# omangin/multimodal

Measured on AMD Instinct MI355X. Metric: nmf_update_iterations_per_sec, higher is better.
Workload: dtype f16 operands, fp32 accumulate; e4m3 ratio tiles and e4m3 W image in the H-numerator product

## Files before the change

### multimodal_amd/csrc/api_loop.hip

```cpp
#include "ctx.hip.h"

namespace klnmf_host {
namespace {

RowPass4Key rowpass4_key(const klnmf_ctx *c, int mode, bool tiles, int grid_y) {
    const bool upd = mode == ROW_UPDATE;
    const bool q8 = upd && c->q8() && tiles;
    const bool ne = q8 && c->ne_loop && !c->big;
    return RowPass4Key{c->KT, 2 * c->KT - c->ks, mode, c->kc >= 0 ? 1 : 0, c->big ? 4 : kWaves4, (upd && grid_y > 1) ? 1 : 0,
                       q8 ? (ne ? 2 : 1) : 0};
}

void launch_rowpass4_kt(klnmf_ctx *c, int mode, const RowPass4Args &a, int grid_x, int grid_y = 1) {
    struct Table {
        void (*slot[kRowPass4Count])(RowPass4Args) = {};
        Table() { KL_RP4_LIST_1(KL_RP4_SLOT) KL_RP4_LIST_2(KL_RP4_SLOT) KL_RP4_LIST_3(KL_RP4_SLOT) }
    };
    static const Table table;
    const RowPass4Key key = rowpass4_key(c, mode, a.base.Qt != nullptr, grid_y);
    if (mode == ROW_UPDATE) c->last_row_ne = key.q8 == 2;
    const int idx = rowpass4_index(key);
    if (idx < 0) fail(KLNMF_ERR_UNSUPP, "ping-pong row pass: 224 < k <= 256 runs on the generation-1 kernel");
    if (!table.slot[idx]) fail(KLNMF_ERR_UNSUPP, "ping-pong row pass: no kernel in slot " + std::to_string(idx));
    hipLaunchKernelGGL(table.slot[idx], dim3(grid_x, grid_y), dim3(64 * key.nw), 0, c->stream, a);
// ... 332 lines not shown
                           NumArray<T, 2>{{(const T *)c->Npart, (const T *)c->Dpart}}, OutSets<T, 2>{{(T *)c->numer, (T *)c->denom}},
                           count, c->nsplit, (const DevState *)c->st);
    else
        hipLaunchKernelGGL((k_sum_partials<T, 1>), dim3(grid_for(count)), dim3(256), 0, c->stream,
                           NumArray<T, 1>{{(const T *)c->Npart}}, OutSets<T, 1>{{(T *)c->numer}}, count, c->nsplit, (const DevState *)c->st);
    HIPCHK(hipGetLastError());
}

template <typename T>
void exact_H(klnmf_ctx *c, bool from_slabs = false) {
    auto rule = [&](auto fac) {
        typedef decltype(fac) Fac;
        typedef NumArray<T, Fac::S> Arr;
        typedef NumSlabs<T, Fac::S> Slabs;
        Arr sums{}, slab0{};
        const T *const psums[2] = {(const T *)c->numer, (const T *)c->denom}, *const pslabs[2] = {(const T *)c->Npart, (const T *)c->Dpart};
        for (int s = 0; s < Fac::S; ++s) { sums.p[s] = psums[s]; slab0.p[s] = pslabs[s]; }
        if (from_slabs) {
            hipLaunchKernelGGL((k_update_H<T, Slabs, Fac>), dim3((unsigned)c->k), dim3(256), 0, c->stream, (T *)c->H,
                               RuleIn<Slabs, Fac>{Slabs{slab0, c->nsplit, c->k * c->f}, fac}, c->f, (const DevState *)c->st);
        } else if (c->hseg_n > 1) {
            hipLaunchKernelGGL((k_update_H_part<T, Fac>), dim3((unsigned)c->hseg_n, (unsigned)c->k), dim3(256), 0, c->stream, (T *)c->H,
                               RuleIn<Arr, Fac>{sums, fac}, c->f, c->hseg, c->hpart, (const DevState *)c->st);
            hipLaunchKernelGGL((k_update_H_norm<T>), dim3((unsigned)c->hseg_n, (unsigned)c->k), dim3(256), 0, c->stream, (T *)c->H,
                               c->f, c->hseg, (const double *)c->hpart, (const DevState *)c->st);
        } else {
            hipLaunchKernelGGL((k_update_H<T, Arr, Fac>), dim3((unsigned)c->k), dim3(256), 0, c->stream, (T *)c->H, RuleIn<Arr, Fac>{sums, fac},
                               c->f, (const DevState *)c->st);
        }
        HIPCHK(hipGetLastError());
    };
    if (c->weighted()) rule(FacDen{});
    else if (c->presence()) rule(FacPresH<T>{(const T *)c->pres_D, (const unsigned char *)c->pres_mod, c->pres_M});
    else rule(FacNum{});
}

#define EXACT_CALL(c, fn, ...)                                         \
    do {                                                               \
        if ((c)->prec == KLNMF_PREC_F64) fn<double>(c, ##__VA_ARGS__); \
        else fn<float>(c, ##__VA_ARGS__);                              \
    } while (0)

}

void launch_monitor(klnmf_ctx *c, bool use8) {
    c->mon_pending = false;
    c->mon_dry_pending = false;
    if (!c->mon_part || !c->sw.q8_monitor || !c->q8_loop) return;
    const bool dry = c->iter_in_loop == 1 && !c->q8();
    if (!dry && !(c->q8() && monitor_due(c->stat_q8_tiles))) return;
    MonArgs a{};
    a.st = c->st; a.Qt = c->Qt; a.VtA = (const _Float16 *)c->VtA; a.W32_old = c->W32[c->cur]; a.H_old = c->H32;
    a.Wb_new = c->Wb[c->cur ^ 1]; a.W8 = (use8 && !dry) ? c->W8 : nullptr; a.w8s = c->w8s; a.part = c->mon_part;
    a.spread = c->mon_spread;
    a.dry = dry ? 1 : 0;
    a.w8tab = (dry && c->W8 != nullptr && c->conv_ran) ? c->w8tab : nullptr;
    a.nrt = c->nrt; a.nct = c->nct; a.kp = c->KP; a.k = (int)c->k; a.wld = (int)w_ld(c->KP); a.w8ld = (int)w8_ld(c->KP);
    a.f_pad = c->f_pad;
    const int tiles = (int)((c->f + 31) / 32);
    a.ct = (int)((c->mon_checks * 5 + 1) % tiles);
    a.ncols = (int)std::min<int64_t>(32, c->f - (int64_t)a.ct * 32);
    a.nrt_data = (int)((c->n + 31) / 32);
    a.nsamp = std::min(2 * kMonBlocks, a.nrt_data) & ~1;
    if (a.nsamp < 2) return;
    a.rot = (int)((c->mon_checks * 7) % a.nrt_data);
    a.eps = (float)(kEpsRatio * c->v_scale);
    hipLaunchKernelGGL(k_q8_monitor, dim3(2 * kMonBlocks), dim3(256), 0, c->stream, a);
    HIPCHK(hipGetLastError());
    c->mon_pending = true;
    c->mon_dry_pending = dry;
    c->mon_ncols = a.ncols;
    c->mon_noise_scale = (float)std::min(0.5, (double)(a.nsamp / 2) * 32.0 / (double)c->n);
    c->mon_checks += 1;
}

bool fused_w8_stage(klnmf_ctx *c) {
    c->conv_ran = false;
    if (!c->W8 || !c->q8_loop) return false;
    const bool measure_only = c->iter_in_loop == 1 && !c->w8_meas;
    if (!measure_only && !c->q8()) return false;
    const bool use8 = !measure_only && c->w8_meas;
    const int groups = c->KP / 8, rpb = std::max(1, 256 / groups);
    const int64_t rows = c->n_pad;
    const int blocks = (int)std::min<int64_t>((rows + rpb - 1) / rpb, kW8Blocks);
    hipLaunchKernelGGL(k_w8_from_wb, dim3(blocks), dim3(256), 0, c->stream, (const opnd_t *)c->Wb[c->cur ^ 1], c->W8, rows,
                       c->KP, (int)w_ld(c->KP), (const float *)c->w8s, (const DevState *)c->st,
                       &c->st->w8_sat, w8_probe_col(c), c->w8tab,
                       ((unsigned)c->sr_launches++ * 0x9E3779B9u + 0x7F4A7C15u) ^ ((unsigned)c->comm_rank * 0xC2B2AE35u));
    HIPCHK(hipGetLastError());
    c->w8_meas = true;
    c->conv_ran = true;
    return use8;
}

void fused_colpass_part(klnmf_ctx *c, const klnmf_ctx::PartCfg &p, bool use8) {
    ColPassQArgs a = colq_part_args(c, p);
    const int grid = p.ncb * p.nchunks;
    EventPair ev{};
    if (c->prof_now) ev = begin_event(c, c->ev_col);
    auto launch_q2 = [&](const ColPassQArgs &g, bool fp8_tiles) {
        switch (c->KT) {
#define KL_PQ2(KTV) case KTV:                                                                                                    \
            if (fp8_tiles) hipLaunchKernelGGL((k_colpass_q2<KTV, KL_COLQ8_NB, 1, 1, KL_COLQ8_PAIR>), dim3(grid), dim3(kThreads), 0, c->stream, g); \
            else hipLaunchKernelGGL((k_colpass_q2<KTV, KL_COLQ_NB>), dim3(grid), dim3(kThreads), 0, c->stream, g);                \
            break;
#define KL_PQ2_BIG(KTV) case KTV:                                                                                                \
            if (fp8_tiles) hipLaunchKernelGGL((k_colpass_q2<KTV, 3, 2, 1, 1>), dim3(grid), dim3(kThreads), 0, c->stream, g);      \
            else hipLaunchKernelGGL((k_colpass_q2<KTV, 3, 2>), dim3(grid), dim3(kThreads), 0, c->stream, g);                      \
            break;
            KL_PQ2(1) KL_PQ2(2) KL_PQ2(3) KL_PQ2(4) KL_PQ2(5) KL_PQ2(6) KL_PQ2(7)
            KL_PQ2_BIG(8) KL_PQ2_BIG(10) KL_PQ2_BIG(12) KL_PQ2_BIG(14) KL_PQ2_BIG(16)
#undef KL_PQ2
#undef KL_PQ2_BIG
            default: fail(KLNMF_ERR_UNSUPP, "stored-ratio column pass: k <= 224 or 256 < k <= 512");
        }
        HIPCHK(hipGetLastError());
    };
    if (use8) {
        a.guard = 1;
        ColPass8Args a8{a, c->W8, c->w8s, w8_probe_col(c) >= 0 ? 1 : 0};
        if (c->KT == 8 && !c->big) fail(KLNMF_ERR_UNSUPP, "fp8 x fp8 column pass: KT = 8 only on the component-split path");
        switch (c->KT) {
#define KL_PQ8X(KTV, NBV, KSV) case KTV:                                                                                          \
            if (a8.probe) hipLaunchKernelGGL((k_colpass_q8x<KTV, NBV, KSV, 1>), dim3(grid), dim3(kThreads), 0, c->stream, a8);     \
            else hipLaunchKernelGGL((k_colpass_q8x<KTV, NBV, KSV, 0>), dim3(grid), dim3(kThreads), 0, c->stream, a8);              \
            break;
            KL_PQ8X(1, KL_COL8_NB, 1) KL_PQ8X(2, KL_COL8_NB, 1) KL_PQ8X(3, KL_COL8_NB, 1) KL_PQ8X(4, KL_COL8_NB, 1)
            KL_PQ8X(5, KL_COL8_NB, 1) KL_PQ8X(6, KL_COL8_NB, 1) KL_PQ8X(7, KL_COL8_NB, 1)
            KL_PQ8X(8, 3, 2) KL_PQ8X(10, 3, 2) KL_PQ8X(12, 3, 2) KL_PQ8X(14, 3, 2) KL_PQ8X(16, 3, 2)
#undef KL_PQ8X
            default: fail(KLNMF_ERR_UNSUPP, "fp8 x fp8 column pass: k <= 224 or 256 < k <= 512");
        }
        HIPCHK(hipGetLastError());
        ColPassQArgs g = a;
        g.guard = 2;
        launch_q2(g, true);
    } else {
        launch_q2(a, c->q8());
    }
    if (c->prof_now) HIPCHK(hipEventRecord(ev.b, c->stream));
}

void launch_post(klnmf_ctx *c, PostMode mode, const klnmf_ctx::PartCfg *parts, int nparts, const LossArgs &la, bool decide,
                 bool use8, bool last_sum) {
    PostArgs a{};
    a.nparts = nparts;
    for (int p = 0; p < nparts; ++p) {
        const klnmf_ctx::PartCfg &q = parts[p];
        a.part[p] = PostPart{c->NpartF + q.slab_off, c->numerF + q.numer_off, (int64_t)c->KP * q.ld, q.ld, q.col0, q.ncols,
                             q.nchunks, q.ct0};
    }
    a.do_sum = mode != POST_RULE;
    a.do_rule = mode != POST_SUM;
    a.do_decide = decide ? 1 : 0;
    a.loss_from_parts = (mode == POST_FULL && la.part != nullptr) ? 1 : 0;
    a.loss_block = (mode == POST_SUM && la.part != nullptr) ? 1 : 0;
    a.w8_block = (a.do_sum && last_sum && c->conv_ran && c->w8tab != nullptr) ? 1 : 0;
    a.last_sum = (a.do_sum && last_sum) ? 1 : 0;
    a.it = (int)(c->iter_in_loop & 1);
    a.mon = MonPost{nullptr, nullptr, kMonMinSpread, kMonMaxCommon, 0, 0.f, kMonThreshold};
    if (a.do_sum && c->mon_pending) {
        a.mon = MonPost{c->mon_part, c->mon_spread, c->sw.mon_min_spread >= 0.f ? c->sw.mon_min_spread : kMonMinSpread,
                        c->sw.mon_threshold > 0.f ? 1.0f : kMonMaxCommon, c->mon_ncols,
                        c->mon_noise_scale, c->sw.mon_threshold > 0.f ? c->sw.mon_threshold : kMonThreshold};
        c->mon_pending = false;
    }
    const int nloss = (a.do_sum && la.part != nullptr)
                          ? (int)std::min<int64_t>(kLossRedMax, std::max<int64_t>(1, (la.count + kLossRedSlice - 1) / kLossRedSlice)) : 0;
    a.loss_red = c->loss_red; a.nloss = nloss; a.inv_c = la.inv_c; a.loss_xchg = c->loss_xchg; a.ne = la.ne; a.cq_on = la.cq_on;
    a.tol_abs = la.tol_abs; a.errors = c->errors; a.cap = c->cap;
    a.st = c->st;
    a.H_old = c->H32; a.H_new = c->H32alt;
    a.Ht4 = c->Ht4; a.hsum = c->hsum; a.tcur = c->tcur; a.t_hs = c->t_hs;
    a.f = c->f; a.f_pad = c->f_pad; a.kp = c->KP; a.k = (int)c->k; a.kc = c->kc;
    a.eps_pad = (float)(kEpsRatio * c->v_scale);
    const bool fix = a.do_sum && c->q8() && c->q8_list != nullptr && c->sw.q8_fixup;
    a.list = fix ? c->q8_list : nullptr;
    a.Qt = c->Qt; a.VtA = (const _Float16 *)c->VtA; a.W32_old = c->W32[c->cur]; a.Wb_new = c->Wb[c->cur ^ 1];
    a.W8 = use8 ? c->W8 : nullptr; a.w8s = c->w8s; a.w8ld = (int)w8_ld(c->KP); a.wld = (int)w_ld(c->KP);
    a.nrt = c->nrt; a.nct = c->nct; a.stages_per_chunk = nparts == 1 ? parts[0].spc : 0; a.eps = (float)(kEpsRatio * c->v_scale);
    a.w8tab = c->w8tab; a.w8s_next = c->w8s_next;
    if (a.do_sum && !fix && c->q8() && c->q8_list != nullptr)
        HIPCHK(hipMemsetAsync(&c->st->q8_list_n, 0, sizeof(int), c->stream));
    if (a.do_sum) {
        SlabSumArgs sa{};
        for (int p = 0; p < nparts; ++p) sa.part[p] = a.part[p];
        sa.nparts = nparts; sa.k = (int)c->k; sa.f_pad = c->f_pad; sa.nloss = nloss;
        sa.loss_part = la.part; sa.loss_count = la.count; sa.loss_red = c->loss_red; sa.st = c->st;
        hipLaunchKernelGGL(k_slab_sum, dim3((unsigned)((c->f_pad + 1023) / 1024), (unsigned)(c->k + nloss)), dim3(256), 0, c->stream, sa);
        HIPCHK(hipGetLastError());
    }
    const int hthreads = c->f_pad >= 4096 ? 1024 : (c->f_pad >= 2048 ? 512 : 256);
    const int blocks = (int)c->k + a.w8_block + a.loss_block;
    hipLaunchKernelGGL(k_post, dim3((unsigned)blocks), dim3(hthreads), 0, c->stream, a);
    HIPCHK(hipGetLastError());
    if (a.do_rule) {
        std::swap(c->H32, c->H32alt);
        c->loop_hswaps += 1;
        c->images_measured = false;
    }
    if (a.w8_block) {
        std::swap(c->w8s, c->w8s_next);
        c->conv_ran = false;
    }
}

bool fp8_poll_due(const klnmf_ctx *c) {
    if (c->is_exact() || !c->q8_loop) return false;
    if (c->mon_dry_pending) return true;
    const bool q8_then = c->iter_in_loop + 1 >= 2 && (!c->big || (c->W8 != nullptr && c->w8_meas));
    return q8_then && monitor_due(c->stat_q8_tiles);
}

// ... 489 lines not shown
```

### multimodal_amd/csrc/colq8x.hip.h

```cpp
#pragma once
#include "colq.hip.h"

#define KL_COL8_PF 1
#define KL_COL8_NB 4

namespace klnmf {

__host__ __device__ constexpr int w8_ld(int kp) { return kp + ((kp / 32) % 2 == 0 ? 32 : 0); }

KL_GLOBAL __launch_bounds__(256) void k_w8_from_wb(const opnd_t *Wb, unsigned char *W8, int64_t rows, int kp, int wld,
                                                    const float *w8s, const DevState *st, int *sat, int probe_col,
                                                    unsigned *tab64, unsigned sr_seed) {
    const int ld8 = w8_ld(kp);
    typedef __attribute__((ext_vector_type(2))) _Float16 f16x2;
    if (st->stop) return;
    KL_FP16_SATURATE();
    __shared__ float red[8][256 / 8 * 8];
    const int groups = kp / 8;
    const int c8 = threadIdx.x % groups, rl = threadIdx.x / groups;
    const int rows_per_block = blockDim.x / groups;
    const int comp = 8 * c8;
    f16x2 inv[4];
    float mx[8];
    int nsat = 0;
#pragma unroll
    for (int u = 0; u < 4; ++u) inv[u] = f16x2{(_Float16)(1.f / w8s[comp + 2 * u]), (_Float16)(1.f / w8s[comp + 2 * u + 1])};
#pragma unroll
    for (int e = 0; e < 8; ++e) mx[e] = 0.f;
    if (rl < rows_per_block) {
        const int64_t stride = (int64_t)gridDim.x * rows_per_block;
        constexpr int U = 4;
        for (int64_t row0 = (int64_t)blockIdx.x * rows_per_block + rl; row0 < rows; row0 += U * stride) {
            opx8 v[U];
#pragma unroll
            for (int q = 0; q < U; ++q) {
                const int64_t row = row0 + q * stride;
                if (row < rows) v[q] = *(const opx8 *)(Wb + row * wld + wb_col((int)(row & 31), comp));
            }
#pragma unroll
            for (int q = 0; q < U; ++q) {
                const int64_t row = row0 + q * stride;
                if (row >= rows) break;
                unsigned out[2];
#pragma unroll
                for (int u = 0; u < 2; ++u) {
                    const f16x2 p0 = f16x2{v[q][4 * u], v[q][4 * u + 1]} * inv[2 * u], p1 = f16x2{v[q][4 * u + 2], v[q][4 * u + 3]} * inv[2 * u + 1];
                    unsigned sd = ((unsigned)row * 0x9E3779B1u) ^ ((unsigned)(comp + 4 * u) * 0x85EBCA6Bu) ^ sr_seed;
                    sd = (sd ^ (sd >> 15)) * 0x2C1B3C6Du;
                    const unsigned r1 = (sd ^ (sd >> 12)) * 0x297A2D39u, r2 = (r1 & 0xffffffu) * 0x6C8E95u + 0x3C6EF35Fu;
                    int w = 0;
                    w = __builtin_amdgcn_cvt_scalef32_sr_fp8_f16(w, p0[0], r1, 1.f, 0);
                    w = __builtin_amdgcn_cvt_scalef32_sr_fp8_f16(w, p0[1], r1 << 7, 1.f, 1);
                    w = __builtin_amdgcn_cvt_scalef32_sr_fp8_f16(w, p1[0], r2, 1.f, 2);
                    w = __builtin_amdgcn_cvt_scalef32_sr_fp8_f16(w, p1[1], r2 << 7, 1.f, 3);
                    const f16x2 top = __builtin_elementwise_max(p0, p1);
                    nsat += (top[0] > (_Float16)448.f || top[1] > (_Float16)448.f) ? ((p0[0] > (_Float16)448.f) + (p0[1] > (_Float16)448.f)
                                                                                     + (p1[0] > (_Float16)448.f) + (p1[1] > (_Float16)448.f)) : 0;
                    out[u] = __builtin_bit_cast(unsigned, w);
                }
                if (probe_col >= comp && probe_col < comp + 8) {
                    const int pc = probe_col - comp;
                    out[pc >> 2] = (out[pc >> 2] & ~(0xffu << (8 * (pc & 3)))) | (0x38u << (8 * (pc & 3)));
                }
                *(uint2 *)(W8 + row * ld8 + comp) = make_uint2(out[0], out[1]);
#pragma unroll
                for (int e = 0; e < 8; ++e) mx[e] = fmaxf(mx[e], (float)v[q][e]);
            }
        }
    }
    if (sat != nullptr && nsat != 0) atomicAdd(sat, nsat);
#pragma unroll
    for (int e = 0; e < 8; ++e) red[e][threadIdx.x] = mx[e];
    __syncthreads();
    if (rl == 0) {
#pragma unroll
        for (int e = 0; e < 8; ++e) {
            float m = red[e][c8];
            for (int q = 1; q < rows_per_block; ++q) m = fmaxf(m, red[e][q * groups + c8]);
            atomicMax(tab64 + (int64_t)(blockIdx.x & 63) * kp + comp + e, __float_as_uint(m));
        }
    }
}

typedef __attribute__((ext_vector_type(2))) int i32x2_t;
template <int OFF>
__device__ __forceinline__ void lds_read_tr8(i32x2_t &dst, unsigned addr) {
    asm volatile("ds_read_b64_tr_b8 %0, %1 offset:%2" : "=v"(dst) : "v"(addr), "n"(OFF));
}

struct ColPass8Args {
    ColPassQArgs q;
    const unsigned char *W8;
    const float *w8s;
    int probe;
};



__device__ __forceinline__ float e4m3_value(unsigned b) {
    const int ex = (int)((b >> 3) & 15u), man = (int)(b & 7u);
    return ex == 0 ? ldexpf((float)man, -9) : ldexpf(1.f + 0.125f * (float)man, ex - 7);
}
template <int KT, int NB, int KSPLIT = 1, int PROBE = 1>
__global__ __launch_bounds__(kThreads, 1) void k_colpass_q8x(ColPass8Args aa) {
    const ColPassQArgs &a = aa.q;
    typedef __attribute__((ext_vector_type(8))) int i32x8;
    typedef i32x2_t i32x2;
    static_assert((KSPLIT == 1 || KSPLIT == 2) && KT % KSPLIT == 0, "wave decomposition");
    constexpr int CTW = kWavesPerWG / KSPLIT;
    constexpr int KTW = KT / KSPLIT;
    constexpr int KP = 32 * KT;
    constexpr int LD8 = w8_ld(KP);
    constexpr int WST = 64 * LD8;
    constexpr int WA = round_up(WST, kGldsRound);
    constexpr int WR = WA / kGldsRound;
    constexpr int QA = CTW * 2 * kQTile8;
    constexpr int OBJ = WA + QA;
    constexpr int QPW = 2 / KSPLIT;
    constexpr int OPS = WR + QPW;
    static_assert(NB >= 3 && NB <= 5 && NB * OBJ <= 160 * 1024, "LDS budget");
    __shared__ __attribute__((aligned(16))) unsigned char o0[OBJ];
    __shared__ __attribute__((aligned(16))) unsigned char o1[OBJ];
    __shared__ __attribute__((aligned(16))) unsigned char o2[OBJ];
    __shared__ __attribute__((aligned(16))) unsigned char o3[NB > 3 ? OBJ : 16];
    __shared__ __attribute__((aligned(16))) unsigned char o4[NB > 4 ? OBJ : 16];
    if (a.st->stop) return;
    if (a.guard == 1 && a.st->w8_sat != 0) return;

    const int tid = threadIdx.x, lane = tid & 63, wave = __builtin_amdgcn_readfirstlane(tid >> 6);
    const int r = lane & 31, h = lane >> 5;
    const int G = gridDim.x;
    int lin = blockIdx.x;
    if ((G & 7) == 0) lin = (blockIdx.x & 7) * (G >> 3) + (blockIdx.x >> 3);
    const int chunk = lin / a.ncb, cb = lin % a.ncb;
    const int ctl = wave % CTW, kh = wave / CTW;
    const int ct_raw = cb * CTW + ctl;
    const bool active = ct_raw < a.nct;
    const int ct = active ? ct_raw : a.nct - 1;
    const int sbeg = chunk * a.stages_per_chunk;
    const int send = min(a.nrt / 2, sbeg + a.stages_per_chunk);
    if (sbeg >= send) {
        if (active) {
            float *np = a.Npart + (int64_t)chunk * KP * a.f_pad + (int64_t)ct * 32 + r;
            for (int c = 32 * KTW * kh + h; c < 32 * KTW * (kh + 1); c += 2) np[(int64_t)c * a.f_pad] = 0.f;
        }
        return;
    }
    const int i16 = lane & 15, half = (lane >> 4) & 1;
    const unsigned off_a = (32 * h + (i16 >> 1)) * LD8 + 16 * half + 8 * (i16 & 1) + 32 * KTW * kh;
    const unsigned off_b = WA + (2 * ctl + h) * kQTile8 + (i16 >> 1) * 32 + 16 * half + 8 * (i16 & 1);

    f32x16 acc[KTW];
#pragma unroll
// ... 25 lines not shown
    float probe_prev = 0.f, probe_max = 0.f;
    unsigned q8_flag = 0u;

    auto compute = [&](unsigned base, int stage_row0) {
        (void)stage_row0;
        i32x2 bq[4];
        static_for<0, 4>([&](auto U) {
            constexpr int u = decltype(U)::value;
            lds_read_tr8<u * 8 * 32>(bq[u], base + off_b);
        });
        constexpr int PF = KL_COL8_PF < KTW ? KL_COL8_PF : (KTW > 1 ? KTW - 1 : 1);
        constexpr int RG = PF + 1;
        i32x2 ring[RG][4];
        auto fetch = [&](auto M) {
            constexpr int m = decltype(M)::value;
            if constexpr (m < KTW) {
                static_for<0, 4>([&](auto U) {
                    constexpr int u = decltype(U)::value;
                    lds_read_tr8<u * 8 * LD8 + 32 * (KTW - 1 - m)>(ring[m % RG][u], base + off_a);
                });
            }
        };
        static_for<0, PF>([&](auto M) { fetch(M); });
        constexpr int young0 = 4 * (PF < KTW ? PF : KTW);
        asm volatile("s_waitcnt lgkmcnt(%4)" : "+v"(bq[0]), "+v"(bq[1]), "+v"(bq[2]), "+v"(bq[3]) : "n"(young0));
        const i32x8 bo = {bq[0][0], bq[0][1], bq[1][0], bq[1][1], bq[2][0], bq[2][1], bq[3][0], bq[3][1]};
        static_for<0, KTW>([&](auto M) {
            constexpr int m = decltype(M)::value;
            fetch(std::integral_constant<int, m + PF>{});
            constexpr int young = 4 * ((m + PF < KTW ? m + PF : KTW - 1) - m);
            asm volatile("s_waitcnt lgkmcnt(%4)" : "+v"(ring[m % RG][0]), "+v"(ring[m % RG][1]), "+v"(ring[m % RG][2]), "+v"(ring[m % RG][3]) : "n"(young));
            const i32x8 ao = {ring[m % RG][0][0], ring[m % RG][0][1], ring[m % RG][1][0], ring[m % RG][1][1],
                              ring[m % RG][2][0], ring[m % RG][2][1], ring[m % RG][3][0], ring[m % RG][3][1]};
            acc[KTW - 1 - m] = __builtin_amdgcn_mfma_scale_f32_32x32x64_f8f6f4(ao, bo, acc[KTW - 1 - m], 0, 0, 0, 127, 0, 127);
            __builtin_amdgcn_sched_barrier(0);
        });
        {
            if constexpr (PROBE != 0) {
                const float now = acc[KTW - 1][15];
                probe_max = fmaxf(probe_max, now - probe_prev);
                probe_prev = now;
            } else {
#pragma unroll
                for (int e = 0; e < 8; ++e) q8_flag |= q8_sat_mask((unsigned)bo[e]);
            }
        }
    };
    auto fence = [&]() {
        __builtin_amdgcn_sched_barrier(0);
        asm volatile("s_waitcnt vmcnt(%0)\n\ts_barrier" ::"n"((NB - 2) * OPS) : "memory");
        __builtin_amdgcn_sched_barrier(0);
    };
    static_for<0, NB - 1>([&](auto I) { stage_in(decltype(I)::value, sbeg + decltype(I)::value); });
    fence();
    for (int s0 = sbeg; s0 < send; s0 += NB) {
        static_for<0, NB>([&](auto I) {
            constexpr int i = decltype(I)::value;
            if (s0 + i < send) {
                stage_in((i + NB - 1) % NB, s0 + i + NB - 1);
                compute(lds_addr(obj(i)), 64 * (s0 + i));
                fence();
            }
        });
    }
    asm volatile("s_waitcnt vmcnt(0)" ::: "memory");
    if (!active) return;
    if (a.q8_list != nullptr && kh == KSPLIT - 1) {
        bool mine;
        if (PROBE != 0) mine = h == 1 && probe_max >= 31.5f;
        else mine = h == 0 && (q8_flag | (unsigned)__shfl_xor((int)q8_flag, 32, 64)) != 0u;
        if (mine) q8_suspect_append(a.st_rw, a.q8_list, chunk, ct, r);
    }
    const int rcol = 8 * ((r >> 2) & 3) + 4 * (r >> 4) + (r & 3);
    float *np = a.Npart + (int64_t)chunk * KP * a.f_pad + (int64_t)ct * 32 + rcol;
#pragma unroll
    for (int m = 0; m < KTW; ++m)
#pragma unroll
        for (int e = 0; e < 16; ++e) {
            const int comp = 32 * (KTW * kh + m) + 8 * (e >> 2) + 4 * h + (e & 3);
            np[(int64_t)comp * a.f_pad] = acc[m][e] * (kQ8Scale * aa.w8s[comp]);
        }
}

}
```

### multimodal_amd/csrc/ctx.hip.h

```cpp
#pragma once
#include <hip/hip_runtime.h>
#include <dlfcn.h>
#include <rccl/rccl.h>

#include <algorithm>
#include <cmath>
#include <cstdio>
#include <cstdlib>
#include <cstring>
#include <functional>
#include <limits>
#include <map>
#include <mutex>
#include <stdexcept>
#include <string>
#include <type_traits>
#include <vector>

#include "../../include/klnmf.h"
#include "stage_chunks.h"
#include "common.hip.h"
#include "exact.hip.h"
#include "weighted.hip.h"
#include "presence.hip.h"
// ... 125 lines not shown
        if (it == free_blocks.end() || it->second.empty()) return nullptr;
        void *p = it->second.back();
        it->second.pop_back();
        held -= cls;
        return p;
    }
    void flush(int device) {
        std::lock_guard<std::mutex> g(mu);
        for (auto &kv : free_blocks) {
            if (kv.first.first != device) continue;
            for (void *p : kv.second) { (void)hipFree(p); held -= kv.first.second; }
            kv.second.clear();
        }
    }
    bool give(int device, size_t cls, void *p) {
        if (cls > ((size_t)64 << 20)) return false;
        std::lock_guard<std::mutex> g(mu);
        if (held + cls > limit()) return false;
        free_blocks[{device, cls}].push_back(p);
        held += cls;
        return true;
    }
};
extern DevBlockCache g_block_cache;

struct DeviceBlocks {
    int device = 0;
    hipStream_t stream = nullptr;
    std::vector<std::pair<void *, size_t>> allocs;
    void *dalloc(size_t bytes, bool zero = true) {
        if (bytes == 0) bytes = 16;
        const size_t cls = DevBlockCache::size_class(bytes);
        void *p = g_block_cache.take(device, cls);
        if (!p) {
            hipError_t e = hipMalloc(&p, cls);
            if (e == hipErrorOutOfMemory) {
                (void)hipGetLastError();
                g_block_cache.flush(device);
                e = hipMalloc(&p, cls);
            }
            HIPCHK(e);
        }
        allocs.push_back({p, cls});
        if (zero) HIPCHK(hipMemsetAsync(p, 0, bytes, stream));
        return p;
    }
    void dfree(void *&p) {
        for (size_t i = 0; i < allocs.size(); ++i) {
            if (allocs[i].first != p) continue;
            if (!g_block_cache.give(device, allocs[i].second, p)) (void)hipFree(p);
            allocs.erase(allocs.begin() + (std::ptrdiff_t)i);
            break;
        }
        p = nullptr;
    }
    void release_all() {
        for (auto &b : allocs)
            if (!g_block_cache.give(device, b.second, b.first)) (void)hipFree(b.first);
        allocs.clear();
    }
};

template <typename Place>
void staged_upload(hipStream_t stream, const void *src, size_t es, int64_t rows, int64_t cols, int64_t ld, Place &&place) {
    const int64_t rows_per = stage_rows_per(rows, ld, es);
    void *d = nullptr;
    HIPCHK(hipMalloc(&d, stage_alloc_bytes(rows_per, ld, es)));
    try {
        stage_walk(rows, cols, ld, es, rows_per, [&](const StageChunk &ch) {
            HIPCHK(hipMemcpyAsync(d, (const char *)src + ch.offset, ch.bytes, hipMemcpyHostToDevice, stream));
            place((const void *)d, ch.r0, ch.rr);
            HIPCHK(hipStreamSynchronize(stream));
        });
    } catch (...) {
        (void)hipFree(d);
        throw;
    }
    (void)hipFree(d);
}

struct DevSwitches {
    int qtile = 0;
    int col8 = -1;
    int ne = -1;
    bool q8_fixup = true;
    bool q8_monitor = true;
    float mon_threshold = 0.f, mon_min_spread = -1.f;
    bool ratio_scale = true;
    bool eps_pad = true;
    int row_split = -1;
    int row_tail = -1;
    int comm_parts = 1;
    bool comm_overlap = true;
    bool comm_single = false;
    int sp_cb = 0, sp_rb = 0;
    int ex_rc = 0, ex_wc = 0;
    int64_t ex_hseg = 0;
    static DevSwitches read() {
        DevSwitches d;
        auto num = [](const char *name, int dflt) { const char *e = std::getenv(name); return e ? std::atoi(e) : dflt; };
        if (num("KLNMF_QTILE", 0) == 16) d.qtile = 16;
        if (num("KLNMF_DEV", 0) == 0) return d;
        d.qtile = num("KLNMF_QTILE", 0);
        d.col8 = num("KLNMF_COL8", -1);
        d.ne = num("KLNMF_NE", -1);
        d.q8_fixup = num("KLNMF_Q8_FIXUP", 1) != 0;
        d.q8_monitor = num("KLNMF_Q8_MONITOR", 1) != 0;
        if (const char *e = std::getenv("KLNMF_MON_THRESHOLD")) d.mon_threshold = (float)std::atof(e);
        if (const char *e = std::getenv("KLNMF_MON_MIN_SPREAD")) d.mon_min_spread = (float)std::atof(e);
        d.ratio_scale = num("KLNMF_RATIO_SCALE", 1) != 0;
        d.eps_pad = num("KLNMF_NO_EPS_PAD", 0) == 0;
        d.row_split = num("KLNMF_ROW_SPLIT", -1);
        d.row_tail = num("KLNMF_ROW_TAIL", -1);
        d.comm_parts = num("KLNMF_COMM_PARTS", 1);
        d.comm_overlap = num("KLNMF_COMM_OVERLAP", 1) != 0;
        d.comm_single = num("KLNMF_COMM_SINGLE", 0) != 0;
        d.sp_cb = num("KLNMF_SP_CB", 0);
        d.sp_rb = num("KLNMF_SP_RB", 0);
        d.ex_rc = std::max(0, num("KLNMF_EX_ROW_CHUNKS", 0));
        d.ex_wc = std::max(0, num("KLNMF_EX_W_CHUNKS", 0));
        d.ex_hseg = std::max(0, num("KLNMF_EX_H_SEG", 0));
        return d;
    }
};

#include "plan.hip.h"

namespace klnmf_host {

struct ContextState : DeviceBlocks {
    int prec = KLNMF_PREC_F64;
    bool own_stream = false;
    int cu_count = 256;
    double ratio_eps = kEpsRatio;
    void *poll_host = nullptr;
    hipEvent_t poll_ev = nullptr;

    bool profiling = false;
    int profile_every = 1;
    int64_t profile_seq = 0;
    std::vector<EventPair> ev_row, ev_col, ev_tail;

    ncclComm_t comm = nullptr;
    int comm_rank = 0, comm_size = 1;
    double *comm_scratch = nullptr;
    hipStream_t comm_stream = nullptr;
    hipEvent_t ev_part[kPostMaxParts] = {}, ev_ar[kPostMaxParts] = {};
};

struct PresenceState {
    int pres_M = 0, pres_dchunks = 0;
    int64_t pres_bounds[kMaxMod + 1] = {};
    void *Pm = nullptr, *pres_S = nullptr, *pres_D = nullptr;
    void *pres_dbounds = nullptr, *pres_mod = nullptr, *pres_Dslab = nullptr;
    bool presence() const { return pres_M > 0; }
    void forget_presence() { *this = PresenceState(); }
};

struct ProblemState : ProblemPlan, PresenceState {
    DevSwitches sw;
    int64_t cap = 0;
    bool have_problem = false;
    int cur = 0;
    int loop_start_cur = 0;
    int64_t loop_hswaps = 0;
    float *loop_h0 = nullptr, *loop_h1 = nullptr;

    DevState *st = nullptr;
    double *errors = nullptr;
    double *loss_xchg = nullptr;
    double2 *loss_red = nullptr;

    void *V = nullptr, *W[2] = {nullptr, nullptr}, *H = nullptr, *Q = nullptr;
    void *Npart = nullptr, *numer = nullptr;
    double *loss_part = nullptr;
    void *Wpart = nullptr;
    void *Om = nullptr, *Dpart = nullptr, *denom = nullptr, *WDpart = nullptr;
    float *x3_hs = nullptr, *x3_qr = nullptr;
    unsigned *x3_xmax = nullptr;
    double *x3_loss = nullptr;

    int64_t *sp_indptr = nullptr, *sp_indices = nullptr, *csc_indptr = nullptr, *csc_rows = nullptr, *csc_perm = nullptr;
    void *sp_data = nullptr, *sp_q = nullptr, *HT = nullptr;
    double *sp_row_loss = nullptr, *sp_wpart = nullptr, *sp_prod = nullptr;
    int *sp_idx32 = nullptr, *csc_rows32 = nullptr, *csc_perm32 = nullptr;
    int64_t *sp_blkptr = nullptr, *csc_blkptr = nullptr;
    double *sp_loss_part = nullptr;
// ... 185 lines not shown
```

Baseline: 215.9.

## Software-pipeline W8 conversion kernel and add opt-in paired fp8 column pass

Rewrites the W-to-fp8 conversion kernel to double-buffer row loads across trips. It uses scalar base offsets and incrementally computed stochastic-rounding seeds, hoists the probe-column mask, and defers saturation counting behind a wave ballot. The per-row max is now tracked on raw f16 bits. A new column-pass kernel variant gives each wave two column tiles sharing one W operand fetch, but it runs only under a dev env switch. The pipelining adds register pressure and relies on static assumptions about row spacing.

```diff
diff --git a/multimodal_amd/csrc/api_loop.hip b/multimodal_amd/csrc/api_loop.hip
--- a/multimodal_amd/csrc/api_loop.hip
+++ b/multimodal_amd/csrc/api_loop.hip
@@ -438,6 +438,7 @@
     const bool use8 = !measure_only && c->w8_meas;
     const int groups = c->KP / 8, rpb = std::max(1, 256 / groups);
     const int64_t rows = c->n_pad;
+    static_assert(kW8Blocks % 16 == 0, "k_w8_from_wb: a thread's rows lie a multiple of 16 apart");
     const int blocks = (int)std::min<int64_t>((rows + rpb - 1) / rpb, kW8Blocks);
     hipLaunchKernelGGL(k_w8_from_wb, dim3(blocks), dim3(256), 0, c->stream, (const opnd_t *)c->Wb[c->cur ^ 1], c->W8, rows,
                        c->KP, (int)w_ld(c->KP), (const float *)c->w8s, (const DevState *)c->st,
@@ -481,10 +482,19 @@
             if (a8.probe) hipLaunchKernelGGL((k_colpass_q8x<KTV, NBV, KSV, 1>), dim3(grid), dim3(kThreads), 0, c->stream, a8);     \
             else hipLaunchKernelGGL((k_colpass_q8x<KTV, NBV, KSV, 0>), dim3(grid), dim3(kThreads), 0, c->stream, a8);              \
             break;
-            KL_PQ8X(1, KL_COL8_NB, 1) KL_PQ8X(2, KL_COL8_NB, 1) KL_PQ8X(3, KL_COL8_NB, 1) KL_PQ8X(4, KL_COL8_NB, 1)
-            KL_PQ8X(5, KL_COL8_NB, 1) KL_PQ8X(6, KL_COL8_NB, 1) KL_PQ8X(7, KL_COL8_NB, 1)
+#define KL_PQ8X1(KTV) case KTV:                                                                                                    \
+            if (c->sw.col8_pair == 1) {                                                                                            \
+                if (a8.probe) hipLaunchKernelGGL((k_colpass_q8x_pair<KTV, KL_COL8_NB, 1>), dim3(grid), dim3(kThreads), 0, c->stream, a8); \
+                else hipLaunchKernelGGL((k_colpass_q8x_pair<KTV, KL_COL8_NB, 0>), dim3(grid), dim3(kThreads), 0, c->stream, a8);   \
+                break;                                                                                                             \
+            }                                                                                                                      \
+            if (a8.probe) hipLaunchKernelGGL((k_colpass_q8x<KTV, KL_COL8_NB, 1, 1>), dim3(grid), dim3(kThreads), 0, c->stream, a8); \
+            else hipLaunchKernelGGL((k_colpass_q8x<KTV, KL_COL8_NB, 1, 0>), dim3(grid), dim3(kThreads), 0, c->stream, a8);         \
+            break;
+            KL_PQ8X(1, KL_COL8_NB, 1) KL_PQ8X1(2) KL_PQ8X1(3) KL_PQ8X1(4) KL_PQ8X1(5) KL_PQ8X1(6) KL_PQ8X1(7)
             KL_PQ8X(8, 3, 2) KL_PQ8X(10, 3, 2) KL_PQ8X(12, 3, 2) KL_PQ8X(14, 3, 2) KL_PQ8X(16, 3, 2)
 #undef KL_PQ8X
+#undef KL_PQ8X1
             default: fail(KLNMF_ERR_UNSUPP, "fp8 x fp8 column pass: k <= 224 or 256 < k <= 512");
         }
         HIPCHK(hipGetLastError());
diff --git a/multimodal_amd/csrc/colq8x.hip.h b/multimodal_amd/csrc/colq8x.hip.h
--- a/multimodal_amd/csrc/colq8x.hip.h
+++ b/multimodal_amd/csrc/colq8x.hip.h
@@ -1,5 +1,6 @@
 #pragma once
 #include "colq.hip.h"
+#include "w8_seed.h"
 
 #define KL_COL8_PF 1
 #define KL_COL8_NB 4
@@ -7,12 +8,52 @@
 namespace klnmf {
 
 __host__ __device__ constexpr int w8_ld(int kp) { return kp + ((kp / 32) % 2 == 0 ? 32 : 0); }
+
+typedef __attribute__((ext_vector_type(2))) _Float16 f16x2;
+typedef __attribute__((ext_vector_type(2))) short s16x2;
+__device__ __forceinline__ s16x2 w8_raw_pair(const opx8 &v, int u) {
+    return __builtin_bit_cast(s16x2, f16x2{v[2 * u], v[2 * u + 1]});
+}
+__device__ __forceinline__ int64_t w8_uniform(int64_t x) {
+    asm("" : "+s"(x));
+    return x;
+}
+struct W8Lane {
+    f16x2 inv[4];
+    unsigned keep[2], put[2];
+};
+__device__ __forceinline__ uint2 w8_convert_row(const opx8 &v, const W8Lane &ln, unsigned sd0, unsigned sd1, f16x2 &top) {
+    unsigned out[2];
+#pragma unroll
+    for (int u = 0; u < 2; ++u) {
+        const f16x2 p0 = f16x2{v[4 * u], v[4 * u + 1]} * ln.inv[2 * u], p1 = f16x2{v[4 * u + 2], v[4 * u + 3]} * ln.inv[2 * u + 1];
+        unsigned r1, r2;
+        w8_seed_mix(u == 0 ? sd0 : sd1, r1, r2);
+        asm("" : "+v"(r1));
+        int w = 0;
+        w = __builtin_amdgcn_cvt_scalef32_sr_fp8_f16(w, p0[0], r1, 1.f, 0);
+        w = __builtin_amdgcn_cvt_scalef32_sr_fp8_f16(w, p0[1], r1 << 7, 1.f, 1);
+        w = __builtin_amdgcn_cvt_scalef32_sr_fp8_f16(w, p1[0], r2, 1.f, 2);
+        w = __builtin_amdgcn_cvt_scalef32_sr_fp8_f16(w, p1[1], r2 << 7, 1.f, 3);
+        top = __builtin_elementwise_max(top, __builtin_elementwise_max(p0, p1));
+        out[u] = (__builtin_bit_cast(unsigned, w) & ln.keep[u]) | ln.put[u];
+    }
+    return make_uint2(out[0], out[1]);
+}
+__device__ __forceinline__ int w8_count_sat(const opx8 &v, const W8Lane &ln) {
+    int n = 0;
+#pragma unroll
+    for (int u = 0; u < 4; ++u) {
+        const f16x2 p = f16x2{v[2 * u], v[2 * u + 1]} * ln.inv[u];
+        n += (p[0] > (_Float16)448.f) + (p[1] > (_Float16)448.f);
+    }
+    return n;
+}
 
 KL_GLOBAL __launch_bounds__(256) void k_w8_from_wb(const opnd_t *Wb, unsigned char *W8, int64_t rows, int kp, int wld,
                                                     const float *w8s, const DevState *st, int *sat, int probe_col,
                                                     unsigned *tab64, unsigned sr_seed) {
     const int ld8 = w8_ld(kp);
-    typedef __attribute__((ext_vector_type(2))) _Float16 f16x2;
     if (st->stop) return;
     KL_FP16_SATURATE();
     __shared__ float red[8][256 / 8 * 8];
@@ -20,55 +61,81 @@
     const int c8 = threadIdx.x % groups, rl = threadIdx.x / groups;
     const int rows_per_block = blockDim.x / groups;
     const int comp = 8 * c8;
-    f16x2 inv[4];
+    W8Lane ln;
+    s16x2 mxp[4];
+    int nsat = 0;
+#pragma unroll
+    for (int u = 0; u < 4; ++u) {
+        ln.inv[u] = f16x2{(_Float16)(1.f / w8s[comp + 2 * u]), (_Float16)(1.f / w8s[comp + 2 * u + 1])};
+        mxp[u] = s16x2{0, 0};
+    }
+#pragma unroll
+    for (int u = 0; u < 2; ++u) {
+        const int pc = probe_col - (comp + 4 * u);
+        const bool here = pc >= 0 && pc < 4;
+        ln.keep[u] = here ? ~(0xffu << (8 * pc)) : ~0u;
+        ln.put[u] = here ? 0x38u << (8 * pc) : 0u;
+    }
+    if (rl < rows_per_block) {
+        constexpr int U = kW8RowsPerTrip;
+        const int64_t stride = (int64_t)gridDim.x * rows_per_block;
+        int64_t brow = (int64_t)blockIdx.x * rows_per_block;
+        const unsigned src_off = 2u * (unsigned)(rl * wld + wb_col((int)((brow + rl) & 31), comp));
+        const unsigned dst_off = (unsigned)(rl * ld8 + comp);
+        const int64_t src_row = 2 * (int64_t)wld, src_q = stride * src_row, dst_q = stride * ld8;
+        const char *const src = (const char *)Wb;
+        int64_t src_o = brow * src_row, dst_o = brow * ld8;
+        W8Seed seed(brow + rl, stride, comp, sr_seed);
+        auto load_trip = [&](opx8(&v)[U], int ahead) {
+#pragma unroll
+            for (int q = 0; q < U; ++q) v[q] = *(const opx8 *)(src + w8_uniform(src_o + (ahead * U + q) * src_q) + src_off);
+        };
+        auto convert_trip = [&](const opx8(&v)[U]) {
+            f16x2 top = f16x2{(_Float16)0.f, (_Float16)0.f};
+#pragma unroll
+            for (int q = 0; q < U; ++q) {
+                *(uint2 *)(W8 + w8_uniform(dst_o + q * dst_q) + dst_off) = w8_convert_row(v[q], ln, seed.at(q, 0), seed.at(q, 1), top);
+#pragma unroll
+                for (int u = 0; u < 4; ++u) mxp[u] = __builtin_elementwise_max(mxp[u], w8_raw_pair(v[q], u));
+            }
+            if (__builtin_amdgcn_ballot_w64(top[0] > (_Float16)448.f || top[1] > (_Float16)448.f) != 0) {
+#pragma unroll
+                for (int q = 0; q < U; ++q) nsat += w8_count_sat(v[q], ln);
+            }
+            brow += U * stride, src_o += U * src_q, dst_o += U * dst_q, seed.next_trip();
+        };
+        if (w8_full_trip(brow, stride, rows_per_block, rows)) {
+            opx8 va[U], vb[U];
+            load_trip(va, 0);
+            for (;;) {
+                if (!w8_full_trip(brow + U * stride, stride, rows_per_block, rows)) { convert_trip(va); break; }
+                load_trip(vb, 1);
+                convert_trip(va);
+                if (!w8_full_trip(brow + U * stride, stride, rows_per_block, rows)) { convert_trip(vb); break; }
+                load_trip(va, 1);
+                convert_trip(vb);
+            }
+        }
+#pragma unroll
+        for (int q = 0; q < U; ++q) {
+            if (brow + q * stride + rl < rows) {
+                const opx8 v = *(const opx8 *)(src + w8_uniform(src_o + q * src_q) + src_off);
+                f16x2 top = f16x2{(_Float16)0.f, (_Float16)0.f};
+                *(uint2 *)(W8 + w8_uniform(dst_o + q * dst_q) + dst_off) = w8_convert_row(v, ln, seed.at(q, 0), seed.at(q, 1), top);
+#pragma unroll
+                for (int u = 0; u < 4; ++u) mxp[u] = __builtin_elementwise_max(mxp[u], w8_raw_pair(v, u));
+                if (top[0] > (_Float16)448.f || top[1] > (_Float16)448.f) nsat += w8_count_sat(v, ln);
+            }
+        }
+    }
+    if (sat != nullptr && nsat != 0) atomicAdd(sat, nsat);
     float mx[8];
-    int nsat = 0;
-#pragma unroll
-    for (int u = 0; u < 4; ++u) inv[u] = f16x2{(_Float16)(1.f / w8s[comp + 2 * u]), (_Float16)(1.f / w8s[comp + 2 * u + 1])};
-#pragma unroll
-    for (int e = 0; e < 8; ++e) mx[e] = 0.f;
-    if (rl < rows_per_block) {
-        const int64_t stride = (int64_t)gridDim.x * rows_per_block;
-        constexpr int U = 4;
-        for (int64_t row0 = (int64_t)blockIdx.x * rows_per_block + rl; row0 < rows; row0 += U * stride) {
-            opx8 v[U];
-#pragma unroll
-            for (int q = 0; q < U; ++q) {
-                const int64_t row = row0 + q * stride;
-                if (row < rows) v[q] = *(const opx8 *)(Wb + row * wld + wb_col((int)(row & 31), comp));
-            }
-#pragma unroll
-            for (int q = 0; q < U; ++q) {
-                const int64_t row = row0 + q * stride;
-                if (row >= rows) break;
-                unsigned out[2];
-#pragma unroll
-                for (int u = 0; u < 2; ++u) {
-                    const f16x2 p0 = f16x2{v[q][4 * u], v[q][4 * u + 1]} * inv[2 * u], p1 = f16x2{v[q][4 * u + 2], v[q][4 * u + 3]} * inv[2 * u + 1];
-                    unsigned sd = ((unsigned)row * 0x9E3779B1u) ^ ((unsigned)(comp + 4 * u) * 0x85EBCA6Bu) ^ sr_seed;
-                    sd = (sd ^ (sd >> 15)) * 0x2C1B3C6Du;
-                    const unsigned r1 = (sd ^ (sd >> 12)) * 0x297A2D39u, r2 = (r1 & 0xffffffu) * 0x6C8E95u + 0x3C6EF35Fu;
-                    int w = 0;
-                    w = __builtin_amdgcn_cvt_scalef32_sr_fp8_f16(w, p0[0], r1, 1.f, 0);
-                    w = __builtin_amdgcn_cvt_scalef32_sr_fp8_f16(w, p0[1], r1 << 7, 1.f, 1);
-                    w = __builtin_amdgcn_cvt_scalef32_sr_fp8_f16(w, p1[0], r2, 1.f, 2);
-                    w = __builtin_amdgcn_cvt_scalef32_sr_fp8_f16(w, p1[1], r2 << 7, 1.f, 3);
-                    const f16x2 top = __builtin_elementwise_max(p0, p1);
-                    nsat += (top[0] > (_Float16)448.f || top[1] > (_Float16)448.f) ? ((p0[0] > (_Float16)448.f) + (p0[1] > (_Float16)448.f)
-                                                                                     + (p1[0] > (_Float16)448.f) + (p1[1] > (_Float16)448.f)) : 0;
-                    out[u] = __builtin_bit_cast(unsigned, w);
-                }
-                if (probe_col >= comp && probe_col < comp + 8) {
-                    const int pc = probe_col - comp;
-                    out[pc >> 2] = (out[pc >> 2] & ~(0xffu << (8 * (pc & 3)))) | (0x38u << (8 * (pc & 3)));
-                }
-                *(uint2 *)(W8 + row * ld8 + comp) = make_uint2(out[0], out[1]);
-#pragma unroll
-                for (int e = 0; e < 8; ++e) mx[e] = fmaxf(mx[e], (float)v[q][e]);
-            }
-        }
-    }
-    if (sat != nullptr && nsat != 0) atomicAdd(sat, nsat);
+#pragma unroll
+    for (int u = 0; u < 4; ++u) {
+        const f16x2 m = __builtin_bit_cast(f16x2, mxp[u]);
+        mx[2 * u] = (float)m[0];
+        mx[2 * u + 1] = (float)m[1];
+    }
 #pragma unroll
     for (int e = 0; e < 8; ++e) red[e][threadIdx.x] = mx[e];
     __syncthreads();
@@ -260,4 +327,186 @@
         }
 }
 
-}
+
+template <int KT, int NB, int PROBE = 1>
+__global__ __launch_bounds__(kThreads, 1) void k_colpass_q8x_pair(ColPass8Args aa) {
+    const ColPassQArgs &a = aa.q;
+    typedef __attribute__((ext_vector_type(8))) int i32x8;
+    typedef i32x2_t i32x2;
+    static_assert(KT >= 2 && KT <= 8, "two halves of the component blocks; 2 x ceil(KT / 2) accumulators per wave");
+    constexpr int CTW = kWavesPerWG;
+    constexpr int K0 = (KT + 1) / 2;
+    constexpr int KP = 32 * KT;
+    constexpr int LD8 = w8_ld(KP);
+    constexpr int WST = 64 * LD8;
+    constexpr int WA = round_up(WST, kGldsRound);
+    constexpr int WR = WA / kGldsRound;
+    constexpr int QA = CTW * 2 * kQTile8;
+    constexpr int OBJ = WA + QA;
+    constexpr int OPS = WR + 2;
+    static_assert(NB >= 3 && NB <= 5 && NB * OBJ <= 160 * 1024, "LDS budget");
+    __shared__ __attribute__((aligned(16))) unsigned char o0[OBJ];
+    __shared__ __attribute__((aligned(16))) unsigned char o1[OBJ];
+    __shared__ __attribute__((aligned(16))) unsigned char o2[OBJ];
+    __shared__ __attribute__((aligned(16))) unsigned char o3[NB > 3 ? OBJ : 16];
+    __shared__ __attribute__((aligned(16))) unsigned char o4[NB > 4 ? OBJ : 16];
+    if (a.st->stop) return;
+    if (a.guard == 1 && a.st->w8_sat != 0) return;
+
+    const int tid = threadIdx.x, lane = tid & 63, wave = __builtin_amdgcn_readfirstlane(tid >> 6);
+    const int r = lane & 31, h = lane >> 5;
+    const int G = gridDim.x;
+    int lin = blockIdx.x;
+    if ((G & 7) == 0) lin = (blockIdx.x & 7) * (G >> 3) + (blockIdx.x >> 3);
+    const int chunk = lin / a.ncb, cb = lin % a.ncb;
+    const int ct_copy = min(cb * CTW + wave, a.nct - 1);
+    const int tp = wave & 3, kh = wave >> 2;
+    const int ct0 = cb * CTW + 2 * tp;
+    const int nact = min(2, max(0, a.nct - ct0));
+    const int sbeg = chunk * a.stages_per_chunk;
+    const int send = min(a.nrt / 2, sbeg + a.stages_per_chunk);
+    const int blk0 = kh == 0 ? 0 : K0, blk1 = kh == 0 ? K0 : KT;
+    if (sbeg >= send) {
+        for (int t = 0; t < nact; ++t) {
+            float *np = a.Npart + (int64_t)chunk * KP * a.f_pad + (int64_t)(ct0 + t) * 32 + r;
+            for (int c = 32 * blk0 + h; c < 32 * blk1; c += 2) np[(int64_t)c * a.f_pad] = 0.f;
+        }
+        return;
+    }
+    const int i16 = lane & 15, half = (lane >> 4) & 1;
+    const unsigned off_a = (32 * h + (i16 >> 1)) * LD8 + 16 * half + 8 * (i16 & 1);
+    const unsigned off_b = WA + (4 * tp + h) * kQTile8 + (i16 >> 1) * 32 + 16 * half + 8 * (i16 & 1);
+
+    const unsigned char *const qt_s = a.Qt + (int64_t)ct_copy * a.nrt * kQTile8;
+    const unsigned t16 = (unsigned)tid * 16u, l16 = (unsigned)lane * 16u;
+    auto obj = [&](int o) -> KL_LDS unsigned char * {
+        return (KL_LDS unsigned char *)(o == 0 ? o0 : o == 1 ? o1 : o == 2 ? o2 : o == 3 ? o3 : o4);
+    };
+    auto lds_addr = [](KL_LDS unsigned char *p) -> unsigned { return (unsigned)(uintptr_t)p; };
+    auto stage_in = [&](int o, int sg) {
+        sg = min(sg, send - 1);
+        const unsigned char *wbase = aa.W8 + (int64_t)sg * WST;
+        const unsigned m0w = lds_addr(obj(o)) + (unsigned)wave * 1024u;
+#pragma unroll
+        for (int rr = 0; rr < WR; ++rr)
+            asm volatile("s_mov_b32 m0, %0\n\ts_nop 0\n\tglobal_load_lds_dwordx4 %1, %2" ::"s"(m0w + rr * kGldsRound), "v"(t16), "s"(wbase + rr * kGldsRound) : "memory");
+        const unsigned char *qbase = qt_s + (int64_t)(2 * sg) * kQTile8;
+#pragma unroll
+        for (int p = 0; p < 2; ++p)
+            asm volatile("s_mov_b32 m0, %0\n\ts_nop 0\n\tglobal_load_lds_dwordx4 %1, %2" ::"s"(lds_addr(obj(o)) + WA + (2 * wave + p) * kQTile8), "v"(l16), "s"(qbase + p * kQTile8) : "memory");
+    };
+    auto fence = [&]() {
+        __builtin_amdgcn_sched_barrier(0);
+        asm volatile("s_waitcnt vmcnt(%0)\n\ts_barrier" ::"n"((NB - 2) * OPS) : "memory");
+        __builtin_amdgcn_sched_barrier(0);
+    };
+    auto run = [&](auto KHc) {
+        constexpr int KH = decltype(KHc)::value;
+        constexpr int KTW = KH == 0 ? K0 : KT - K0;
+        constexpr int BASE = KH == 0 ? 0 : K0;
+        f32x16 acc0[KTW], acc1[KTW];
+#pragma unroll
+        for (int m = 0; m < KTW; ++m)
+#pragma unroll
+            for (int e = 0; e < 16; ++e) acc0[m][e] = acc1[m][e] = 0.f;
+        float probe_prev0 = 0.f, probe_max0 = 0.f, probe_prev1 = 0.f, probe_max1 = 0.f;
+        unsigned q8_flag0 = 0u, q8_flag1 = 0u;
+        auto compute = [&](unsigned base) {
+            i32x2 bq[8];
+            static_for<0, 4>([&](auto U) {
+                constexpr int u = decltype(U)::value;
+                lds_read_tr8<u * 8 * 32>(bq[u], base + off_b);
+            });
+            static_for<0, 4>([&](auto U) {
+                constexpr int u = decltype(U)::value;
+                lds_read_tr8<u * 8 * 32 + 2 * kQTile8>(bq[4 + u], base + off_b);
+            });
+            constexpr int PF = KL_COL8_PF < KTW ? KL_COL8_PF : (KTW > 1 ? KTW - 1 : 1);
+            constexpr int RG = PF + 1;
+            i32x2 ring[RG][4];
+            auto fetch = [&](auto M) {
+                constexpr int m = decltype(M)::value;
+                if constexpr (m < KTW) {
+                    static_for<0, 4>([&](auto U) {
+                        constexpr int u = decltype(U)::value;
+                        lds_read_tr8<u * 8 * LD8 + 32 * (BASE + KTW - 1 - m)>(ring[m % RG][u], base + off_a);
+                    });
+                }
+            };
+            static_for<0, PF>([&](auto M) { fetch(M); });
+            constexpr int young0 = 4 * (PF < KTW ? PF : KTW);
+            asm volatile("s_waitcnt lgkmcnt(%8)"
+                         : "+v"(bq[0]), "+v"(bq[1]), "+v"(bq[2]), "+v"(bq[3]), "+v"(bq[4]), "+v"(bq[5]), "+v"(bq[6]), "+v"(bq[7])
+                         : "n"(young0));
+            const i32x8 bo0 = {bq[0][0], bq[0][1], bq[1][0], bq[1][1], bq[2][0], bq[2][1], bq[3][0], bq[3][1]};
+            const i32x8 bo1 = {bq[4][0], bq[4][1], bq[5][0], bq[5][1], bq[6][0], bq[6][1], bq[7][0], bq[7][1]};
+            static_for<0, KTW>([&](auto M) {
+                constexpr int m = decltype(M)::value;
+                fetch(std::integral_constant<int, m + PF>{});
+                constexpr int young = 4 * ((m + PF < KTW ? m + PF : KTW - 1) - m);
+                asm volatile("s_waitcnt lgkmcnt(%4)" : "+v"(ring[m % RG][0]), "+v"(ring[m % RG][1]), "+v"(ring[m % RG][2]), "+v"(ring[m % RG][3]) : "n"(young));
+                const i32x8 ao = {ring[m % RG][0][0], ring[m % RG][0][1], ring[m % RG][1][0], ring[m % RG][1][1],
+                                  ring[m % RG][2][0], ring[m % RG][2][1], ring[m % RG][3][0], ring[m % RG][3][1]};
+                acc0[KTW - 1 - m] = __builtin_amdgcn_mfma_scale_f32_32x32x64_f8f6f4(ao, bo0, acc0[KTW - 1 - m], 0, 0, 0, 127, 0, 127);
+                acc1[KTW - 1 - m] = __builtin_amdgcn_mfma_scale_f32_32x32x64_f8f6f4(ao, bo1, acc1[KTW - 1 - m], 0, 0, 0, 127, 0, 127);
+                __builtin_amdgcn_sched_barrier(0);
+            });
+            if constexpr (KH == 1) {
+                if constexpr (PROBE != 0) {
+                    const float now0 = acc0[KTW - 1][15], now1 = acc1[KTW - 1][15];
+                    probe_max0 = fmaxf(probe_max0, now0 - probe_prev0);
+                    probe_max1 = fmaxf(probe_max1, now1 - probe_prev1);
+                    probe_prev0 = now0;
+                    probe_prev1 = now1;
+                } else {
+#pragma unroll
+                    for (int e = 0; e < 8; ++e) {
+                        q8_flag0 |= q8_sat_mask((unsigned)bo0[e]);
+                        q8_flag1 |= q8_sat_mask((unsigned)bo1[e]);
+                    }
+                }
+            }
+        };
+        static_for<0, NB - 1>([&](auto I) { stage_in(decltype(I)::value, sbeg + decltype(I)::value); });
+        fence();
+        for (int s0 = sbeg; s0 < send; s0 += NB) {
+            static_for<0, NB>([&](auto I) {
+                constexpr int i = decltype(I)::value;
+                if (s0 + i < send) {
+                    stage_in((i + NB - 1) % NB, s0 + i + NB - 1);
+                    compute(lds_addr(obj(i)));
+                    fence();
+                }
+            });
+        }
+        asm volatile("s_waitcnt vmcnt(0)" ::: "memory");
+        if (nact == 0) return;
+        if (KH == 1 && a.q8_list != nullptr) {
+            bool mine0, mine1;
+            if (PROBE != 0) {
+                mine0 = h == 1 && probe_max0 >= 31.5f;
+                mine1 = h == 1 && probe_max1 >= 31.5f;
+            } else {
+                mine0 = h == 0 && (q8_flag0 | (unsigned)__shfl_xor((int)q8_flag0, 32, 64)) != 0u;
+                mine1 = h == 0 && (q8_flag1 | (unsigned)__shfl_xor((int)q8_flag1, 32, 64)) != 0u;
+            }
+            if (mine0) q8_suspect_append(a.st_rw, a.q8_list, chunk, ct0, r);
+            if (mine1 && nact > 1) q8_suspect_append(a.st_rw, a.q8_list, chunk, ct0 + 1, r);
+        }
+        const int rcol = 8 * ((r >> 2) & 3) + 4 * (r >> 4) + (r & 3);
+        float *np = a.Npart + (int64_t)chunk * KP * a.f_pad + (int64_t)ct0 * 32 + rcol;
+#pragma unroll
+        for (int m = 0; m < KTW; ++m)
+#pragma unroll
+            for (int e = 0; e < 16; ++e) {
+                const int comp = 32 * (BASE + m) + 8 * (e >> 2) + 4 * h + (e & 3);
+                const float sc = kQ8Scale * aa.w8s[comp];
+                np[(int64_t)comp * a.f_pad] = acc0[m][e] * sc;
+                if (nact > 1) np[(int64_t)comp * a.f_pad + 32] = acc1[m][e] * sc;
+            }
+    };
+    if (kh == 0) run(std::integral_constant<int, 0>{});
+    else run(std::integral_constant<int, 1>{});
+}
+
+}
diff --git a/multimodal_amd/csrc/ctx.hip.h b/multimodal_amd/csrc/ctx.hip.h
--- a/multimodal_amd/csrc/ctx.hip.h
+++ b/multimodal_amd/csrc/ctx.hip.h
@@ -231,6 +231,7 @@
 struct DevSwitches {
     int qtile = 0;
     int col8 = -1;
+    int col8_pair = 0;
     int ne = -1;
     bool q8_fixup = true;
     bool q8_monitor = true;
@@ -252,6 +253,7 @@
         if (num("KLNMF_DEV", 0) == 0) return d;
         d.qtile = num("KLNMF_QTILE", 0);
         d.col8 = num("KLNMF_COL8", -1);
+        d.col8_pair = num("KLNMF_COL8_PAIR", 0);
         d.ne = num("KLNMF_NE", -1);
         d.q8_fixup = num("KLNMF_Q8_FIXUP", 1) != 0;
         d.q8_monitor = num("KLNMF_Q8_MONITOR", 1) != 0;
diff --git a/multimodal_amd/csrc/w8_seed.h b/multimodal_amd/csrc/w8_seed.h
--- /dev/null
+++ b/multimodal_amd/csrc/w8_seed.h
@@ -0,0 +1,39 @@
+#pragma once
+#include <cstdint>
+
+#if defined(__HIPCC__)
+#define KL_W8_HD __host__ __device__ __forceinline__
+#else
+#define KL_W8_HD inline
+#endif
+
+namespace klnmf {
+
+constexpr int kW8RowsPerTrip = 4;
+
+struct W8Seed {
+    unsigned row_term;
+    unsigned step;
+    unsigned comp_term[2];
+
+    KL_W8_HD static unsigned closed(int64_t row, int comp4, unsigned sr_seed) {
+        return ((unsigned)row * 0x9E3779B1u) ^ ((unsigned)comp4 * 0x85EBCA6Bu) ^ sr_seed;
+    }
+    KL_W8_HD W8Seed(int64_t row0, int64_t stride, int comp, unsigned sr_seed)
+        : row_term((unsigned)row0 * 0x9E3779B1u), step((unsigned)stride * 0x9E3779B1u),
+          comp_term{((unsigned)comp * 0x85EBCA6Bu) ^ sr_seed, ((unsigned)(comp + 4) * 0x85EBCA6Bu) ^ sr_seed} {}
+    KL_W8_HD unsigned at(int q, int u) const { return (row_term + (unsigned)q * step) ^ comp_term[u]; }
+    KL_W8_HD void next_trip() { row_term += (unsigned)kW8RowsPerTrip * step; }
+};
+
+KL_W8_HD void w8_seed_mix(unsigned sd, unsigned &r1, unsigned &r2) {
+    sd = (sd ^ (sd >> 15)) * 0x2C1B3C6Du;
+    r1 = (sd ^ (sd >> 12)) * 0x297A2D39u;
+    r2 = (r1 & 0xffffffu) * 0x6C8E95u + 0x3C6EF35Fu;
+}
+
+KL_W8_HD bool w8_full_trip(int64_t brow, int64_t stride, int rpb, int64_t rows) {
+    return brow + (kW8RowsPerTrip - 1) * stride + rpb <= rows;
+}
+
+}
```

New measurement: 216.6, median of 6. About the same (+0.3%).
